# Molecolab-Pisa/diaglib

Measured on AMD Instinct MI355X. Metric: eigensolver GFLOP/s + iters-to-converge, n=2e6 m=8 Davidson, 1/2/4/8 GPU, higher is better.
Workload: dtype f64; 1 GPU; davidson n=2000000 roots=8 n_max=13 max_dav=20 tol=2e-13 operator=diag(i+1)+0.5*W*W^T(rank 4) guess=unit callbacks=device; workload_key=davidson n=2000000 roots=8 n_max=13 max_dav=20 guess=unit, iters=9, matvec_cols=105, restarts=0, converged=True, rows_per_gpu=2000000

## Files before the change

### diaglib_amd/csrc/hip_engine.hip

```cpp
#include <hip/hip_runtime.h>
#include <rccl/rccl.h>
#include <algorithm>
#include <cmath>
#include <cstdio>
#include <cstdlib>
#include <type_traits>
#include <utility>
#include <cstring>
#include <ctime>
#include <map>
#include <set>
#include <vector>
#include "dla_internal.h"
#include "hip_owned.h"
#include "hip_plans.h"

using namespace dla_plans;

typedef double v4d __attribute__((ext_vector_type(4)));
typedef double v2d __attribute__((ext_vector_type(2)));

template <int V> struct VecOf;
template <> struct VecOf<1> { typedef double type; };
template <> struct VecOf<2> { typedef v2d type; };
// ... 106 lines not shown
  };
  bool want[TLW][KT];
  bool any_want = false;
#pragma unroll
  for (int t = 0; t < TLW; ++t)
#pragma unroll
    for (int q = 0; q < KT; ++q) {
      want[t][q] = !a.lower || (xg * TLW + t >= ug * KT + q);
      any_want = any_want || want[t][q];
    }
  auto mfma_chunk = [&](const vec_t (&xd)[TLW][RSTEP], const vec_t (&ud)[KT][RSTEP]) {
#pragma unroll
    for (int s = 0; s < RSTEP; ++s)
#pragma unroll
      for (int e = 0; e < VEC; ++e)
#pragma unroll
        for (int t = 0; t < TLW; ++t)
#pragma unroll
          for (int q = 0; q < KT; ++q)
            if (want[t][q])
              acc[t][q] = __builtin_amdgcn_mfma_f64_16x16x4f64(vget<VEC>(xd[t][s], e), vget<VEC>(ud[q][s], e),
                                                               acc[t][q], 0, 0, 0);
  };
  if (!any_want) ch = (1LL << 62);
  if constexpr (PREFETCH) {
    if (ch < nfull) {
      load_chunk(ch, xv, uv);
      for (; ch + stride < nfull; ch += stride) {
        vec_t xn[TLW][RSTEP], un[KT][RSTEP];
        load_chunk(ch + stride, xn, un);
        mfma_chunk(xv, uv);
#pragma unroll
        for (int t = 0; t < TLW; ++t)
#pragma unroll
          for (int s = 0; s < RSTEP; ++s) xv[t][s] = xn[t][s];
#pragma unroll
        for (int q = 0; q < KT; ++q)
#pragma unroll
          for (int s = 0; s < RSTEP; ++s) uv[q][s] = un[q][s];
      }
      mfma_chunk(xv, uv);
      ch += stride;
    }
  } else {
    for (; ch < nfull; ch += stride) {
      load_chunk(ch, xv, uv);
      mfma_chunk(xv, uv);
    }
  }
  if (ch == nfull && nfull * CH < n) {
    const long long rbase = nfull * CH;
#pragma unroll
    for (int s = 0; s < RSTEP; ++s) {
      const bool ok = rbase + 4 * VEC * s + VEC * g < n;
#pragma unroll
      for (int q = 0; q < KT; ++q) {
        uv[q][s] = vzero<VEC>();
        if (ok) uv[q][s] = *(const vec_t*)(up[q] + rbase + 4 * VEC * s);
      }
#pragma unroll
      for (int t = 0; t < TLW; ++t) {
        xv[t][s] = vzero<VEC>();
        if (ok) xv[t][s] = *(const vec_t*)(xp[t] + rbase + 4 * VEC * s);
      }
    }
    mfma_chunk(xv, uv);
  }

  __shared__ double red[4][256];
  double* pout = a.partial + ((size_t)blockIdx.y * gridDim.x + blockIdx.x) * (size_t)(TLW * KT) * 256;
#pragma unroll
  for (int t = 0; t < TLW; ++t)
#pragma unroll
    for (int q = 0; q < KT; ++q) {
#pragma unroll
      for (int r = 0; r < 4; ++r) red[wave][r * 64 + lane] = acc[t][q][r];
      __syncthreads();
      double s = ((red[0][threadIdx.x] + red[1][threadIdx.x]) + red[2][threadIdx.x]) + red[3][threadIdx.x];
      pout[(size_t)(t * KT + q) * 256 + threadIdx.x] = s;
      __syncthreads();
    }
}

template <int TLW, int KT, int NT = 1, int R = 16, int SELF = 0, int QT = 0, int LOW = 0, int WP = 0>
__global__ __launch_bounds__(256) void gram_lds_kernel(GramArgs a)
{
  DLA_PREDICATED(a);
  static_assert(!WP || (QT == 0 && LOW == 0 && KT <= 3 && (KT == 1 || (!SELF && R == 16))), "pending factor: up to three U tiles");
  static_assert(WP != 2 || (KT == 1 && !SELF), "projection sweep: one U tile beside the X tiles");
  constexpr int UU = (WP && !SELF) ? KT * (KT + 1) / 2 : 0;
  constexpr int NSLOT = TLW * KT + UU;
  constexpr int RS = R + 2;
  constexpr int LPC = R / 2;
  constexpr int CPI = 64 / LPC;
  constexpr int NC = SELF ? 16 * TLW : 16 * (TLW + KT);
  constexpr int UOFF = SELF ? 0 : 16 * TLW;
  constexpr int NI = NC / CPI;
  extern __shared__ __attribute__((aligned(16))) double glds[];
  const int lane = threadIdx.x & 63, wave = threadIdx.x >> 6;
  double* my = glds + (size_t)wave * NC * RS;
  const int c = lane & 15, g = lane >> 4;
  const int li = lane % LPC, lc = lane / LPC;
  const int xg = blockIdx.y % a.passes_x, ug = blockIdx.y / a.passes_x;
  const long long n = a.n;

  v4d acc[TLW][KT];
  bool want[TLW][KT];
  bool any_want = false;
  unsigned tile_used = 0;
#pragma unroll
  for (int t = 0; t < TLW; ++t)
#pragma unroll
    for (int q = 0; q < KT; ++q) {
      acc[t][q] = (v4d){0.0, 0.0, 0.0, 0.0};
      const int xt = xg * TLW + t, ut = ug * KT + q;
      want[t][q] = (16 * xt < a.l) && (16 * ut < a.k) && (LOW ? (t >= q) : (!a.lower || xt >= ut));
      any_want = any_want || want[t][q];
      if (want[t][q]) tile_used |= (1u << t) | (1u << (SELF ? q : TLW + q));
    }
  const double* cp[NI];
  unsigned skip = 0;
#pragma unroll
  for (int j = 0; j < NI; ++j) {
    const int sc = CPI * j + lc;
    if (!(tile_used & (1u << ((CPI * j) / 16)))) skip |= 1u << j;
    if (sc < 16 * TLW) {
      int col = xg * TLW * 16 + sc;
      if (xg * TLW * 16 + CPI * j >= a.l) skip |= 1u << j;
      col = col < a.l ? col : a.l - 1;
      cp[j] = a.x + (size_t)col * (size_t)n + 2 * li;
    } else {
      int col = ug * KT * 16 + (sc - 16 * TLW);
      if (ug * KT * 16 + (CPI * j - 16 * TLW) >= a.k) skip |= 1u << j;
      col = col < a.k ? col : a.k - 1;
      cp[j] = a.u + (size_t)col * (size_t)n + 2 * li;
    }
  }
  if (a.noskip & 1) skip = 0;
  long long rmul[NI];
#pragma unroll
  for (int j = 0; j < NI; ++j) {
    rmul[j] = 1;
    if (skip & (1u << j)) { rmul[j] = 0; cp[j] = a.x; }
  }
  const int i4 = lane & 3;
  double accq[SELF ? KT : TLW][QT > 0 ? QT : 1];
#pragma unroll
  for (int t = 0; t < (SELF ? KT : TLW); ++t)
#pragma unroll
    for (int qq = 0; qq < (QT > 0 ? QT : 1); ++qq) accq[t][qq] = 0.0;
  v4d accuu[UU > 0 ? UU : 1];
#pragma unroll
  for (int e = 0; e < (UU > 0 ? UU : 1); ++e) accuu[e] = (v4d){0.0, 0.0, 0.0, 0.0};
  double wa[WP == 1 ? KT * (KT + 1) / 2 : 1][WP == 1 ? 4 : 1];
  double ca[WP == 2 ? 4 * (TLW + 1) : 1];
  if constexpr (WP == 2) {
#pragma unroll
    for (int s = 0; s < 4 * (TLW + 1); ++s) {
      const int sc = 4 * s + g;
      const int row = sc < 16 * TLW ? (sc < a.l ? sc : -1) : (sc - 16 * TLW < a.k ? a.l + sc - 16 * TLW : -1);
      ca[s] = row >= 0 ? a.cx[(size_t)row * 16 + c] : 0.0;
    }
  }
  if constexpr (WP == 1) {
    const int k4w = ((a.k + 3) / 4) * 4;
#pragma unroll
    for (int q = 0; q < KT; ++q)
#pragma unroll
      for (int p = 0; p <= q; ++p)
#pragma unroll
        for (int s = 0; s < 4; ++s) {
          const int pp = 16 * p + 4 * s + g;
          double v = (pp == 16 * q + c) ? 1.0 : 0.0;
          if (a.wp) v = (KT == 1) ? a.wp[pp * 16 + c] : (pp < k4w ? a.wp[((size_t)q * k4w + pp) * 16 + c] : 0.0);
          wa[q * (q + 1) / 2 + p][s] = v;
        }
  }
  typedef VecOf<2>::type vec_t;
  vec_t stg[NI];
  auto load_tile = [&](long long tile) {
    const long long r0 = tile * R;
    if constexpr (LOW) {
#pragma unroll
      for (int j = 0; j < NI; ++j) {
        const int sc = CPI * j + lc;
        const bool isx = sc < 16 * TLW;
        int col = isx ? sc : sc - 16 * TLW;
        col = col < a.l ? col : a.l - 1;
        const double* base = isx ? a.x : a.u;
        const bool pin = (isx ? CPI * j : CPI * j - 16 * TLW) >= a.l;
        stg[j] = pload<2, NT>(pin ? a.x : base + (size_t)col * (size_t)n + 2 * li + r0);
      }
    } else {
#pragma unroll
      for (int j = 0; j < NI; ++j) stg[j] = pload<2, NT>(cp[j] + r0 * rmul[j]);
    }
  };
  auto stage_tile = [&]() {
#pragma unroll
    for (int j = 0; j < NI; ++j) lds_store2(my + (size_t)(CPI * j + lc) * RS + 2 * li, stg[j]);
  };
  constexpr int KF = (QT > 0 && !SELF) ? KT - 1 : KT;
  constexpr int TF = (QT > 0 && SELF) ? TLW - 1 : TLW;
  auto apply_w = [&](long long r0w, bool rows_ok) {
    if constexpr (WP) {
      if (WP == 1 && a.wp == nullptr && a.uw == nullptr) return;
      double* ut = my + (size_t)UOFF * RS + c;
      if constexpr (WP == 2) {
        v4d d[R / 16];
#pragma unroll
        for (int h = 0; h < R / 16; ++h) d[h] = (v4d){0.0, 0.0, 0.0, 0.0};
#pragma unroll
        for (int s = 0; s < 4 * (TLW + 1); ++s)
#pragma unroll
          for (int h = 0; h < R / 16; ++h)
            d[h] = __builtin_amdgcn_mfma_f64_16x16x4f64(ca[s], lds_load1(my + (size_t)(4 * s + g) * RS + c + 16 * h), d[h], 0, 0, 0);
        __builtin_amdgcn_wave_barrier();
#pragma unroll
        for (int h = 0; h < R / 16; ++h)
#pragma unroll
          for (int r = 0; r < 4; ++r) lds_store1(ut + (size_t)(g + 4 * r) * RS + 16 * h, d[h][r]);
      } else if constexpr (KT == 1) {
        double uin[R / 16][4];
#pragma unroll
        for (int h = 0; h < R / 16; ++h)
#pragma unroll
          for (int s = 0; s < 4; ++s) uin[h][s] = lds_load1(ut + (size_t)(4 * s + g) * RS + 16 * h);
        v4d d[R / 16];
#pragma unroll
        for (int h = 0; h < R / 16; ++h) d[h] = (v4d){0.0, 0.0, 0.0, 0.0};
#pragma unroll
        for (int s = 0; s < 4; ++s)
#pragma unroll
          for (int h = 0; h < R / 16; ++h) d[h] = __builtin_amdgcn_mfma_f64_16x16x4f64(wa[0][s], uin[h][s], d[h], 0, 0, 0);
#pragma unroll
        for (int h = 0; h < R / 16; ++h)
#pragma unroll
          for (int r = 0; r < 4; ++r) lds_store1(ut + (size_t)(g + 4 * r) * RS + 16 * h, d[h][r]);
      } else {
        double uin[KT][4];
#pragma unroll
        for (int p = 0; p < KT; ++p)
#pragma unroll
          for (int s = 0; s < 4; ++s) uin[p][s] = lds_load1(ut + (size_t)(16 * p + 4 * s + g) * RS);
        v4d d[KT];
#pragma unroll
        for (int q = 0; q < KT; ++q) {
          d[q] = (v4d){0.0, 0.0, 0.0, 0.0};
#pragma unroll
          for (int p = 0; p <= q; ++p)
#pragma unroll
            for (int s = 0; s < 4; ++s) d[q] = __builtin_amdgcn_mfma_f64_16x16x4f64(wa[q * (q + 1) / 2 + p][s], uin[p][s], d[q], 0, 0, 0);
        }
        __builtin_amdgcn_wave_barrier();
#pragma unroll
        for (int q = 0; q < KT; ++q)
#pragma unroll
          for (int r = 0; r < 4; ++r) lds_store1(ut + (size_t)(16 * q + g + 4 * r) * RS, d[q][r]);
      }
      __builtin_amdgcn_wave_barrier();
      if (a.uw != nullptr && rows_ok) {
#pragma unroll
        for (int j = (16 * (SELF ? 0 : TLW)) / CPI; j < NI; ++j) {
          const int uc = CPI * j + lc - UOFF;
          if (uc < a.k) pstore<2, 0>(a.uw + (size_t)uc * (size_t)n + r0w + 2 * li, *(const lds_v2f64*)(my + (size_t)(CPI * j + lc) * RS + 2 * li));
        }
      }
    }
  };
  auto mfma_tile = [&]() {
#pragma unroll
    for (int s4 = 0; s4 < R / 4; ++s4) {
      double uf[KT];
#pragma unroll
      for (int q = 0; q < (SELF ? KT : KF); ++q) uf[q] = lds_load1(my + (size_t)(UOFF + 16 * q + c) * RS + 4 * s4 + g);
      if constexpr (UU > 0) {
#pragma unroll
        for (int qi = 0; qi < KT; ++qi)
#pragma unroll
          for (int qj = 0; qj <= qi; ++qj)
            accuu[qi * (qi + 1) / 2 + qj] = __builtin_amdgcn_mfma_f64_16x16x4f64(uf[qi], uf[qj], accuu[qi * (qi + 1) / 2 + qj], 0, 0, 0);
      }
      double uq[QT > 0 ? QT : 1];
      if constexpr (QT > 0 && !SELF) {
#pragma unroll
        for (int qq = 0; qq < QT; ++qq) uq[qq] = lds_load1(my + (size_t)(UOFF + 16 * KF + 4 * qq + i4) * RS + 4 * s4 + g);
      }
#pragma unroll
      for (int t = 0; t < TF; ++t) {
        const double xf = lds_load1(my + (size_t)(16 * t + c) * RS + 4 * s4 + g);
#pragma unroll
        for (int q = 0; q < KF; ++q)
          if (want[t][q]) acc[t][q] = __builtin_amdgcn_mfma_f64_16x16x4f64(xf, uf[q], acc[t][q], 0, 0, 0);
        if constexpr (QT > 0 && !SELF) {
#pragma unroll
          for (int qq = 0; qq < QT; ++qq)
            if (want[t][KT - 1]) accq[t][qq] = mfma_quarter(xf, uq[qq], accq[t][qq]);
        }
      }
      if constexpr (QT > 0 && SELF) {
#pragma unroll
        for (int qq = 0; qq < QT; ++qq) {
          const double xq = lds_load1(my + (size_t)(16 * TF + 4 * qq + i4) * RS + 4 * s4 + g);
#pragma unroll
          for (int q = 0; q < KT; ++q) accq[q][qq] = mfma_quarter(xq, uf[q], accq[q][qq]);
        }
      }
    }
  };
  const long long nfull = n / R;
  const long long stride = (long long)gridDim.x * 4;
  long long tile = (long long)blockIdx.x * 4 + wave;
  if (!any_want) tile = (1LL << 62);
  if (tile < nfull) {
    load_tile(tile);
    for (;;) {
      stage_tile();
      __builtin_amdgcn_wave_barrier();
      const long long next = tile + stride;
      if (next < nfull) load_tile(next);
      apply_w(tile * R, true);
      mfma_tile();
      __builtin_amdgcn_wave_barrier();
      tile = next;
      if (next >= nfull) break;
    }
  }
  if (tile == nfull && nfull * R < n) {
    const long long r0 = nfull * R;
    const bool ok = r0 + 2 * li < n;
#pragma unroll
    for (int j = 0; j < NI; ++j) {
      stg[j] = vzero<2>();
      if (ok) stg[j] = *(const vec_t*)(cp[j] + r0 * rmul[j]);
    }
    stage_tile();
    __builtin_amdgcn_wave_barrier();
    apply_w(r0, ok);
    mfma_tile();
    __builtin_amdgcn_wave_barrier();
  }

  __syncthreads();
  double* red = glds;
  double* pout = a.partial + ((size_t)blockIdx.y * gridDim.x + blockIdx.x) * (size_t)NSLOT * 256;
  if constexpr (UU > 0) {
#pragma unroll
    for (int e = 0; e < UU; ++e) {
#pragma unroll
      for (int r = 0; r < 4; ++r) red[wave * 256 + r * 64 + lane] = accuu[e][r];
      __syncthreads();
      pout[(size_t)(TLW * KT + e) * 256 + threadIdx.x] = ((red[threadIdx.x] + red[256 + threadIdx.x]) + red[512 + threadIdx.x]) + red[768 + threadIdx.x];
      __syncthreads();
    }
  }
#pragma unroll
  for (int t = 0; t < TLW; ++t)
#pragma unroll
    for (int q = 0; q < KT; ++q) {
      if (LOW && t < q) {
        pout[(size_t)(t * KT + q) * 256 + threadIdx.x] = 0.0;
        continue;
      }
      if (QT > 0 && !SELF && q == KT - 1) {
#pragma unroll
        for (int r = 0; r < 4; ++r) red[wave * 256 + r * 64 + lane] = 0.0;
#pragma unroll
        for (int qq = 0; qq < QT; ++qq) red[wave * 256 + ((lane >> 2) & 3) * 64 + 16 * g + 4 * qq + i4] = accq[t][qq];
      } else if (QT > 0 && SELF && t == TLW - 1) {
#pragma unroll
        for (int r = 0; r < 4; ++r) red[wave * 256 + r * 64 + lane] = r < QT ? accq[q][r < QT ? r : 0] : 0.0;
      } else {
#pragma unroll
        for (int r = 0; r < 4; ++r) red[wave * 256 + r * 64 + lane] = acc[t][q][r];
      }
      __syncthreads();
      double sum = ((red[threadIdx.x] + red[256 + threadIdx.x]) + red[512 + threadIdx.x]) + red[768 + threadIdx.x];
      pout[(size_t)(t * KT + q) * 256 + threadIdx.x] = sum;
      __syncthreads();
    }
}

struct GemmArgs {
  const double* x;
  const double* cpk;
  double* z;
  double* gpart;
  long long n;
  int l, l4, k;
  const int* phase;
  int want;
  int xpf;
};

struct GemmArgsInl {
  const double* x;
  double* z;
  double* gpart;
  long long n;
  int l, l4, k;
  const int* phase;
  int want;
  int xpf;
  double cin[256];
};
__device__ __forceinline__ const double* packed_c(const GemmArgs& a) { return a.cpk; }
__device__ __forceinline__ const double* packed_c(const GemmArgsInl& a) { return a.cin; }

template <int KT, int VEC, int MODE, typename ARGS, bool GRAM = false, int NT = (MODE == 2 ? 0 : 1), int PIPE = (KT >= 2 ? 2 : 0), int ZPAD = 9,
          int QT = 0, int RTP = 2>
__global__ __launch_bounds__(256) void gemm_kernel(ARGS a)
{
  DLA_PREDICATED(a);
  constexpr int RT = RTP;
  constexpr int RG = 16 * VEC;
  constexpr int WT = RT * RG;
  extern __shared__ __attribute__((aligned(16))) double cs[];
  typedef typename VecOf<VEC>::type vec_t;
  const long long n = a.n;
// ... 3170 lines not shown
  int reduce_and_sum(int cls, double* c, double* c_host, int nblk, int l, int k, int tlw, int kt, int px, int n_out, int extra, int ldc,
                     StepOut& out)
  {
    Rode rode;
    {
      Scope s2(this, cls, 0.0, 0.0, "gram_reduce_kernel");
      const int groups = reduce_groups(nblk);
      { const int stl = ensure_lvl2(sizeof(double) * (size_t)n_out * groups * 256); if (stl) return stl; }
      if (n_out > 4096) { err = "gram: too many output tiles"; return DLA_ERR_ARG; }
      GramReduceArgs ra{d_partial, d_lvl2, d_ticket, c, c_host, nblk, l, k, tlw, kt, px,
                        lc.phase, lc.want, 0, n_out, d_ticket + 4096, OrthoTailArgs{}, P2PArgs{}, extra, ldc};
      rode = launch_reduce(ra, dim3(n_out, groups));
    }
    HIPCHK(hipGetLastError());
    out.tail_fused = rode.tail;
    if (lc.in_chunk) return DLA_OK;
    return allreduce_dev(c, (ldc ? ldc : l) * k, 0, h_small, out, rode.exchange);
  }
  void launch_tail_kernel(const OrthoTailArgs& ta)
  {
    if (ta.fold) DLA_LAUNCH(ortho_tail16_kernel, dim3(1), dim3(256), 0, st, ta);
    else DLA_LAUNCH(ortho_tail_kernel, dim3(1), dim3(64), 0, st, ta);
  }

  int launch_op(int op, int n, int m, int k, const double* x, const double* bx, double* u, bool publish, int fold)
  {
    OrthoTailArgs tail{d_ost, h_ost.dev(), d_small, d_wpk, d_wfull, d_cpk2, op, m, k, m > 0 ? 1 : 0, ortho_maxit, publish ? 1 : 0,
                       fold, knobs.lead_full() ? 0 : 1, d_xug, d_wst, d_dbg, lc.xw ? 1 : 0};
    if ((fold == 1 && op == OP_GRAMX) || op == OP_XW || op == OP_COMBOX) tail.gsrc = d_xug;
    tail.x3 = lc.x3 ? 1 : 0;
    tail.gp = knobs.first_factor_source();
    tail.dmat = (policy.basis_exact && fold && m > 0 && dmat_nontrivial && dmat_cols == m && m <= DMAT_LD) ? d_dmat : nullptr;
    tail.dmat_ld = DMAT_LD;
    tail.drop_final = (policy.drop_final && m > 0) ? 1 : 0;
    tail.t_host = (tail.drop_final && policy.publish_pending && m + k <= PEND_ROWS) ? h_tpend.dev() : nullptr;
    tail.t_seq = t_seq;
    tail.drop_tol = policy.drop_tol;
    tail.drop_stol = policy.drop_stol;
    StepOut out;
    int stc = DLA_OK;
    {
      LaunchCtx step = lc;
      step.fuse_tail = p2p.on ? !knobs.exchange_own_launch() : (nranks <= 1 && !comm);
      step.tail = tail;
      step.phase = &d_ost->phase;
      step.want = (op == OP_GRAMX) ? (int)OP_GRAM_UU : (lc.x3 && op == OP_COMBO) ? (int)OP_COMBOX : op;
      CtxScope scope(this, step);
      int blocks = 0;
      switch (op) {
        case OP_GRAM_UU: stc = gram_dev_once(n, k, u, k, u, DLA_OP_GRAM, false, out); break;
        case OP_XU:      stc = gram_dev_once(n, m, bx, k, u, DLA_OP_GRAM, false, out); break;
        case OP_GRAMX:
          stc = fold == 1 ? gram_wp_once(n, m, bx, k, u, nullptr, nullptr, out) : gram_dev_once(n, m + k, x, k, u, DLA_OP_GRAM, false, out);
          break;
        case OP_XW:      stc = gram_wp_once(n, m, bx, k, u, d_wpk, u, out); break;
        case OP_GRAMW:   stc = gram_wp_once(n, 0, nullptr, k, u, d_wpk, nullptr, out); break;
        case OP_TRMMG:
        case OP_TRMMC:
          stc = gemm_chunk(n, 0, k, u, k, nullptr, 0, u, 2, DLA_OP_TRMM, &blocks, d_wpk);
          if (!stc) stc = fused_reduce(k, blocks, out);
          break;
        case OP_COMBO:
          stc = gemm_chunk(n, 0, m + k, x, k, nullptr, 0, u, 0, DLA_OP_GEMM, &blocks, d_cpk2);
          if (!stc) stc = fused_reduce(k, blocks, out);
          break;
        case OP_FINAL:   stc = gemm_chunk(n, 0, k, u, k, nullptr, 0, u, 2, DLA_OP_TRMM, nullptr, d_wpk); break;
        case OP_COMBOX:  stc = gram_wp_once(n, m, bx, k, u, nullptr, u, out, d_cpk2); break;
        case OP_CLOSE:   stc = gemm_chunk(n, 0, m + k, x, k, nullptr, 0, u, 0, DLA_OP_GEMM, nullptr, d_cpk2); break;
        default: err = "ortho_chain: bad op"; stc = DLA_ERR_ARG;
      }
    }
    if (stc || out.tail_fused) return stc;
    if (comm && !p2p.on && d_red_small) {
      if (out.summed_at) tail.gsrc = out.summed_at;
      tail.xug = d_red_xug;
    }
    Scope s(this, DLA_OP_GRAM, 0.0, 0.0, fold ? "ortho_tail16_kernel" : "ortho_tail_kernel");
    launch_tail_kernel(tail);
    HIPCHK(hipGetLastError());
    return DLA_OK;
  }

  template <int TLW, int KT, int R>
  int launch_gram_wp(const GramArgs& a, dim3 grid, bool self)
  {
    if (a.cx != nullptr) {
      if constexpr (KT == 1) {
        auto kfn = gram_lds_kernel<TLW, 1, 1, R, 0, 0, 0, 2>;
        const size_t lds = gram_lds_bytes(TLW, 1, R, false, false);
        if (!raise_lds((const void*)kfn, lds)) return DLA_ERR_RUNTIME;
        DLA_LAUNCH(kfn, grid, dim3(256), lds, st, a);
        return DLA_OK;
      }
      err = "gram_wp: the projection sweep takes one-tile blocks"; return DLA_ERR_ARG;
    }
    if (self) {
      if constexpr (TLW == 1 && KT == 1) {
        auto kfn = gram_lds_kernel<1, 1, 1, 32, 1, 0, 0, 1>;
        const size_t lds = gram_lds_bytes(1, 1, 32, true, false);
        DLA_LAUNCH(kfn, grid, dim3(256), lds, st, a);
      }
      return DLA_OK;
    }
    auto kfn = gram_lds_kernel<TLW, KT, 1, R, 0, 0, 0, 1>;
    const size_t lds = gram_lds_bytes(TLW, KT, R, false, false);
    if (!raise_lds((const void*)kfn, lds)) return DLA_ERR_RUNTIME;
    DLA_LAUNCH(kfn, grid, dim3(256), lds, st, a);
    return DLA_OK;
  }
  int gram_wp_once(int n, int m, const double* x, int k, const double* u, const double* wp, double* uw, StepOut& out, const double* cx = nullptr)
  {
    out = StepOut{};
    const bool self = (m == 0);
    if (cx != nullptr && (self || uw == nullptr || wp != nullptr || k > 16)) { err = "gram_wp: bad projection sweep"; return DLA_ERR_ARG; }
    if (k > 48 || (self && k > 16)) { err = "gram_wp: block too wide"; return DLA_ERR_ARG; }
    const WpPlan p = wp_plan(env(), n, m, k, cx != nullptr);
    const int tlw = p.tlw, kt = p.kt, passes = p.passes, blocks = p.blocks, extra = p.extra, slots = p.slots;
    int stc = ensure_partial(sizeof(double) * (size_t)passes * blocks * slots * 256);
    if (stc) return stc;
    stc = ensure_small(sizeof(double) * (size_t)k * k);
    if (stc) return stc;
    if (!self && (m + k) * k > XUG_DOUBLES) { err = "gram_wp: basis too wide for the chain's buffer"; return DLA_ERR_ARG; }
    if (uw != nullptr && passes != 1) { err = "gram_wp: the storing sweep takes one pass"; return DLA_ERR_ARG; }
    GramArgs a{self ? u : x, u, d_partial, (long long)n, self ? k : m, k, passes, 0, lc.phase, lc.want, 0, wp, uw, cx};
    dim3 grid(blocks, passes);
    {
      Scope s(this, cx ? DLA_OP_GEMM : DLA_OP_GRAM, 8.0 * (double)n * (double)(m + k + (uw ? k : 0)),
              2.0 * (double)n * (m + k) * k + ((wp || cx) ? 1.0 * (double)n * k * k : 0.0) + (cx ? 2.0 * (double)n * m * k : 0.0), p.name());
      int r_ = DLA_ERR_RUNTIME;
      if (!first_instance<std::size(WP_TILES)>([&](auto i) {
            constexpr WpTile s = WP_TILES[decltype(i)::value];
            if (tlw != s.tlw || kt != s.kt || p.R != s.R) return false;
            r_ = launch_gram_wp<s.tlw, s.kt, s.R>(a, grid, self);
            return true;
          }))
        err = "gram_wp: no kernel instance";
      if (r_) return r_;
    }
    const int n_out = self ? 1 : passes * tlw * kt + extra;
    return reduce_and_sum(DLA_OP_GRAM, self ? d_small : d_xug, nullptr, blocks, self ? k : m, k, tlw, kt, passes, n_out, extra, self ? k : m + k, out);
  }

  struct ChainRun {
    bool active = false;
    int n = 0, m = 0, k = 0, fold = 0;
    bool vsx = false;
    const double *x = nullptr, *bx = nullptr;
    double* u = nullptr;
    ChainShape shape;
    bool xw = false;
    bool x3 = false;
    bool lean = false;
    std::vector<int> plan, launched;
    std::vector<SpecRec> recs;
  } run;

  DeviceBuffer<double> d_dmat;
  std::vector<std::vector<double>> h_dcols;
  int dmat_cols = 0;
  bool dmat_nontrivial = false;
  int basis_state(int m) const override { return m <= 0 ? 0 : dmat_cols != m ? -1 : dmat_nontrivial ? 1 : 0; }
  int basis_capacity() const override { return DMAT_LD; }
  bool basis_exact_ok() const override { return !hook && !local_only && !knobs.no_exact_basis() && lds_limit > (size_t)128 * 1024; }
  int basis_dd(int m, int k, double* xu, int ld) override
  {
    if (!policy.basis_exact || m <= 0) return DLA_OK;
    if (dmat_cols != m) { err = "ortho_vs_x: the copy of the caller's pending blocks does not describe this basis (dla_basis_sync after every block)"; return DLA_ERR_ARG; }
    if (!dmat_nontrivial) return DLA_OK;
    std::vector<double> y(m);
    for (int j = 0; j < k; ++j) {
      double* s = xu + (size_t)j * ld;
      for (int r = 0; r < m; ++r) {
        const double* dr = h_dcols[r].data();
        double acc = 0.0;
        for (int i = 0; i <= r; ++i) acc += dr[i] * s[i];
        y[r] = acc;
      }
      for (int i = 0; i < m; ++i) s[i] = 0.0;
      for (int q = 0; q < m; ++q) {
        const double* dq = h_dcols[q].data();
        const double yq = y[q];
        for (int i = 0; i <= q; ++i) s[i] += dq[i] * yq;
      }
    }
    return DLA_OK;
  }
  int basis_sync(int m, int k, const double* dmat, int ld) override
  {
    if (k <= 0) { dmat_cols = 0; dmat_nontrivial = false; h_dcols.clear(); return DLA_OK; }
    if (m != dmat_cols) { err = "basis_sync: the blocks of D arrive in order (" + std::to_string(dmat_cols) + " columns known, block starts at " + std::to_string(m) + ")"; return DLA_ERR_ARG; }
    h_dcols.resize((size_t)m + k);
    for (int j = 0; j < k; ++j) {
      std::vector<double>& col = h_dcols[(size_t)m + j];
      col.resize((size_t)m + j + 1);
      for (int i = 0; i <= m + j; ++i) {
        const double v = dmat[(size_t)i + (size_t)(m + j) * ld];
        col[i] = v;
        if (v != (i == m + j ? 1.0 : 0.0)) dmat_nontrivial = true;
      }
    }
    dmat_cols = m + k;
    if (m + k > DMAT_LD) return DLA_OK;
    bind();
    { const int stz = reserve_zeroed(d_dmat, (size_t)DMAT_LD * DMAT_LD); if (stz) return stz; }
    double* h = nullptr;
    int slot = 0;
    const size_t bytes = sizeof(double) * (size_t)k * DMAT_LD;
    const int stc = stage_slot(bytes, &h, &slot);
    if (stc) return stc;
    std::memset(h, 0, bytes);
    for (int j = 0; j < k; ++j) std::memcpy(h + (size_t)j * DMAT_LD, h_dcols[(size_t)m + j].data(), sizeof(double) * (size_t)(m + j + 1));
    return stage_commit(slot, bytes, d_dmat + (size_t)m * DMAT_LD);
  }

  int pending_block(int m, int k, double* p, int ldp, int* applied) override
  {
// ... 230 lines not shown
          std::printf("    op %llu (err est %.2e, max|G-I| %.2e, max|X^T U| %.2e (col sq %.2e), chol %llu cycles = %.2f GHz): kernel entry->tail %.2f us | G load %.2f | chol+inv %.2f | norms %.2f | products+stores %.2f | decide %.2f | publish %.2f | assemble %.2f\n",
                      q[9], 2.2e-16 * rc * rc, gdev, sdev, csq, q[11], us(1, 2) > 0 ? (double)q[11] / (us(1, 2) * 1e3) : 0.0, us(8, 0), us(0, 1), us(1, 2), us(2, 3), us(3, 4), us(4, 5), us(5, 6), us(6, 7));
        }
        (void)hipMemset(d_dbg, 0, sizeof(unsigned long long) * 48 * 16);
      }
    }
    {
      const int nlog = std::min(sres.nops, 48);
      ChainDone cd;
      cd.launched.swap(launched); cd.recs.swap(recs);
      std::copy(sres.log, sres.log + nlog, cd.log);
      cd.nlog = nlog; cd.n = n; cd.k = k;
      unaccounted.push_back(std::move(cd));
      if (sres.status == OST_DONE && sres.nops <= 48) { hist.assign(sres.log, sres.log + nlog); last_k = hist; }
    }
    if (sres.status == OST_DONE && policy.publishes() && vsx && h_tpend[PEND_HDR] == (double)t_seq) t_pending_k = k;
    rep->handled = 1;
    rep->status = sres.status;
    rep->growth = sres.growth;
    rep->outer_its = sres.it_outer;
    rep->macro_its = sres.macro_total;
    rep->shifts = sres.shifts;
    return DLA_OK;
  }

  DeviceBuffer<int> d_bgo; MappedHostBuffer<int> h_bstat; DeviceBuffer<double> d_wpk_b;
  int b_seq = 0;
  int b_ortho_ahead(int n, int k, double* u, double* bu, bool behind_chain, int* handled) override
  {
    *handled = 0;
    if (k <= 0 || k > 48 || hook || local_only || knobs.no_b_ortho_ahead()) return DLA_OK;
    bind();
    { const int stz = reserve_zeroed(d_bgo, 1); if (stz) return stz; }
    HIPCHK(h_bstat.reserve(1));
    HIPCHK(d_wpk_b.reserve(3 * 48 * 16));
    int stc = ensure_chain_buffers();
    if (stc) return stc;
    StepOut gram_out;
    stc = gram_dev(n, k, u, k, bu, gram_out);
    if (stc) return stc;
    b_seq = b_seq >= 1000000 ? 1 : b_seq + 1;
    *h_bstat = 0;
    {
      Scope s(this, DLA_OP_GRAM, 0.0, 0.0, "bortho_tail_kernel");
      BOrthoTailArgs ta{d_ost, d_small, d_wpk_b, k, behind_chain ? 1 : 0, b_seq, d_bgo, h_bstat.dev()};
      DLA_LAUNCH(bortho_tail_kernel, dim3(1), dim3(64), 0, st, ta);
      HIPCHK(hipGetLastError());
    }
    {
      LaunchCtx behind = lc;
      behind.phase = d_bgo; behind.want = b_seq;
      CtxScope scope(this, behind);
      stc = gemm_chunk(n, 0, k, u, k, nullptr, 0, u, 2, DLA_OP_TRMM, nullptr, d_wpk_b);
      if (!stc) stc = gemm_chunk(n, 0, k, bu, k, nullptr, 0, bu, 2, DLA_OP_TRMM, nullptr, d_wpk_b);
    }
    if (stc) return stc;
    *handled = 1;
    return DLA_OK;
  }
  int b_ortho_ahead_status() override
  {
    const int v = *(volatile int*)h_bstat;
    return v == b_seq ? 1 : (v == -b_seq ? -1 : 0);
  }

  template <int TLW, int KT, int R>
  int launch_gram_lds(const GramArgs& a, dim3 grid, const GramPlan& p)
  {
#define GLK(SELF_, Q)                                                                                          \
    do {                                                                                                      \
      auto kfn = gram_lds_kernel<TLW, KT, 1, R, SELF_, Q>;                                                    \
      const size_t lds = gram_lds_bytes(TLW, KT, R, SELF_, false);                                            \
      if (!raise_lds((const void*)kfn, lds)) return DLA_ERR_RUNTIME;                                          \
      DLA_LAUNCH(kfn, grid, dim3(256), lds, st, a);                                                   \
      return DLA_OK;                                                                                          \
    } while (0)
    if constexpr (TLW == KT) {
      if (p.self) {
        if constexpr (KT >= 2) { if (p.qt == 1) GLK(1, 1); if (p.qt == 2) GLK(1, 2); }
        GLK(1, 0);
      }
    }
    if constexpr (KT >= 2) { if (p.qt == 1) GLK(0, 1); if (p.qt == 2) GLK(0, 2); }
    GLK(0, 0);
#undef GLK
  }
  template <int T>
  int launch_gram_low(const GramArgs& a, dim3 grid, const GramPlan& p)
  {
    auto kfn = gram_lds_kernel<T, T, 1, 16, 0, 0, 1>;
    const size_t lds = gram_lds_bytes(T, T, 16, false, true);
    if (!raise_lds((const void*)kfn, lds)) return DLA_ERR_RUNTIME;
    DLA_LAUNCH(kfn, grid, dim3(256), lds, st, a);
    return DLA_OK;
  }
  template <int TLW, int KT>
  int launch_gram(const GramArgs& a, dim3 grid, const GramPlan& p)
  {
    if constexpr (KT <= 3) {
      if (p.lds) {
        if constexpr (gram_can32(TLW, KT)) { if (p.rows == 32) return launch_gram_lds<TLW, KT, 32>(a, grid, p); }
        return launch_gram_lds<TLW, KT, 16>(a, grid, p);
      }
    }
    if constexpr (!gram_direct_instance(TLW, KT)) {
      err = "gram: width without a direct-load instance";
      return DLA_ERR_RUNTIME;
    } else {
      constexpr int RS = gram_rs(TLW, KT);
      if (p.vec2) DLA_LAUNCH((gram_kernel<TLW, KT, 2, RS>), grid, dim3(256), 0, st, a);
      else      DLA_LAUNCH((gram_kernel<TLW, KT, 1, RS>), grid, dim3(256), 0, st, a);
      return DLA_OK;
    }
  }

  int gram_dev(int n, int l, const double* x, int k, const double* u, StepOut& out, int cls = DLA_OP_GRAM, bool lower = false)
  {
    return with_lds_retry([&]() { return gram_dev_once(n, l, x, k, u, cls, lower, out); });
  }
  int gram_dev_once(int n, int l, const double* x, int k, const double* u, int cls, bool lower, StepOut& out)
  {
    out = StepOut{};
    const GramPlan p = gram_plan(env(), n, l, k, x == u, peers_even && ((uintptr_t)x | (uintptr_t)u) % 16 == 0, lower);
    const int tlw = p.tlw, kt = p.kt, passes = p.passes, blocks_per_pass = p.blocks_per_pass;
    out.lower_only = p.self;
    const int slots = tlw * kt;
    int stc = ensure_partial(sizeof(double) * (size_t)passes * blocks_per_pass * slots * 256);
    if (stc) return stc;
    stc = ensure_small(sizeof(double) * (size_t)l * k);
    if (stc) return stc;
    GramArgs a{x, u, d_partial, (long long)n, l, k, p.px, p.lower ? 1 : 0, lc.phase, lc.want, knobs.gram_load_pads() ? 1 : 0};
    dim3 grid(blocks_per_pass, passes);
    {
      const bool same = (x == u) && (l == k);
      Scope s(this, cls, 8.0 * (double)n * (same ? (double)k : (double)(l + k)), 2.0 * (double)n * l * k, p.name());
      int r_ = DLA_ERR_RUNTIME;
      const bool hit = p.low_single ? first_instance<std::size(GRAM_LOW_TILES)>([&](auto i) {
                                        constexpr int T = GRAM_LOW_TILES[decltype(i)::value];
                                        if (tlw != T) return false;
                                        r_ = launch_gram_low<T>(a, grid, p);
                                        return true;
                                      })
                                    : first_instance<std::size(GRAM_TILES)>([&](auto i) {
                                        constexpr GramTile s = GRAM_TILES[decltype(i)::value];
                                        if (tlw != s.tlw || kt != s.kt) return false;
                                        r_ = launch_gram<s.tlw, s.kt>(a, grid, p);
                                        return true;
                                      });
      if (!hit) err = "gram: no kernel instance";
      if (r_) return r_;
    }
    return reduce_and_sum(cls, d_small + lc.small_off, lc.phase ? nullptr : h_small.dev() + lc.small_off, blocks_per_pass, l, k, tlw, kt, p.px,
                          passes * slots, 0, 0, out);
  }

  Event ev_chunk;
  bool gram_chunks_ok(int n, int l, int k) override
  {
    (void)n;
    return !hook && !comm && !p2p.on && (local_only || nranks <= 1) && l > 0 && k > 0 && lc.phase == nullptr;
  }
  int gram_chunk(int n, int l, const double* x, int k_total, int c0, int kc, const double* u_chunk) override
  {
    if (c0 == 0) { int stc = ensure_small(sizeof(double) * (size_t)l * k_total); if (stc) return stc; }
    HIPCHK(ev_chunk.ensure(hipEventDisableTiming));
    HIPCHK(hipEventRecord(ev_chunk, st_up));
// ... 1173 lines not shown
```

### diaglib_amd/csrc/hip_plans.h

```cpp
#pragma once
#include <algorithm>
#include <cstddef>
#include <cstdio>
#include <iterator>
#include <string>
#include <tuple>
#include <vector>
#include "dla_internal.h"

namespace dla_plans {

struct Knobs {
  int tune[8] = {0, 0, 0, 0, 0, 0, 0, 0};
  void set(int i, int v) { if (i >= 0 && i < 8) tune[i] = v; }
  int get(int i) const { return (i >= 0 && i < 8) ? tune[i] : 0; }
  int ritz_pipe_depth() const { return tune[0] == 1 ? 0 : tune[0] == 4 ? 4 : -1; }
  bool ritz_p_separate() const { return tune[0] == 5; }
  bool no_ritz2() const { return tune[0] == 6; }
  int ritz_grid_factor() const { return tune[1] > 0 ? tune[1] : 1; }
  int gemm_pipe_depth() const { return tune[2] == 1 ? 0 : tune[2] == 4 ? 4 : -1; }
  int gemm_blocks_per_cu() const { return tune[3] > 0 ? tune[3] : 0; }
  int gram_blocks_override() const { return tune[4] > 0 ? tune[4] : 0; }
  bool wp_one_block_per_cu() const { return tune[4] == -1; }
  bool direct_gram() const { return tune[5] == 2; }
  bool fenced_reduce() const { return tune[5] == 3; }
  bool poll_stream() const { return tune[6] == 2; }
  bool host_loop() const { return tune[6] == 3; }
  bool exchange_own_launch() const { return tune[6] == 4; }
  bool no_mfma_kxk() const { return tune[6] == 5; }
  bool no_pending_factor() const { return tune[6] == 6; }
  bool no_wide_gramx() const { return tune[6] == 7 || tune[6] == 8; }
  bool lead_full() const { return tune[6] == 7; }
  bool no_wide_xw() const { return tune[6] == 9; }
  bool wide_xw_three_tiles() const { return tune[6] == 10; }
  bool no_b_ortho_ahead() const { return tune[6] == 11; }
  bool five_sweep() const { return tune[6] == 12; }
  bool three_pass_always() const { return tune[6] == 13; }
  bool mode5_as_mode4() const { return tune[6] == 14; }
  bool no_exact_basis() const { return host_loop() || no_mfma_kxk() || mode5_as_mode4(); }
  int first_factor_source() const { return tune[6] == 15 ? 0 : tune[6] == 16 ? 2 : 1; }
  bool keep_closing_launches() const { return tune[6] == 17; }
  bool no_quarter_tiles() const { return tune[7] == 1; }
  bool gram_load_pads() const { return tune[7] == 2; }
  bool narrow_gram_passes() const { return tune[7] == 3; }
  bool no_next_tile_prefetch() const { return tune[7] == 4; }
  bool fused3_two_row_groups() const { return tune[7] == 5; }
  bool no_low_single() const { return tune[7] == 8; }
  bool own_copy_kernel() const { return tune[7] == 9; }
  int reduce_group_size() const { return tune[7] == 22 ? 16 : tune[7] == 23 ? 64 : 32; }
};

constexpr int DMAT_LD = 320, XUG_DOUBLES = 640 * 16, P2P_MAX_DOUBLES = 16384, PEND_ROWS = 640;

struct PlanEnv { int ncu; size_t lds_limit; const Knobs& knobs; };

template <typename... A>
inline std::string plan_name(const char* fmt, A... a)
{
  char kn[96];
  std::snprintf(kn, sizeof kn, fmt, a...);
  return kn;
}

inline int quarter_tiles(const PlanEnv& env, int k, bool vec2)
{
  const int kt = (k + 15) / 16, rem = k - 16 * (kt - 1);
  return (vec2 && kt >= 2 && kt <= 3 && rem <= 8 && !env.knobs.no_quarter_tiles()) ? (rem + 3) / 4 : 0;
}
inline int blocks_per_cu(size_t lds) { return lds > 80 * 1024 ? 1 : lds > 40 * 1024 ? 2 : 4; }

struct GramTile { int tlw, kt; };
constexpr GramTile GRAM_TILES[] = {
  {1, 1}, {2, 1}, {3, 1}, {4, 1}, {5, 1}, {6, 1}, {7, 1}, {8, 1}, {10, 1}, {12, 1},
  {1, 2}, {2, 2}, {3, 2}, {4, 2}, {5, 2}, {6, 2}, {7, 2}, {8, 2},
  {1, 3}, {2, 3}, {3, 3}, {4, 3}, {5, 3}, {6, 3}, {7, 3},
  {1, 4}, {2, 4}, {3, 4}};
constexpr bool gram_direct_instance(int tlw, int kt)
{
  return !(tlw == 5 || tlw == 7 || tlw == 10 || (tlw == 12 && kt > 1) || (tlw == 3 && kt >= 2 && kt <= 3) || (tlw >= 5 && kt == 3) ||
           (tlw >= 7 && kt == 2));
}
constexpr int GRAM_LOW_TILES[] = {4, 5, 6, 7};
struct WpTile { int tlw, kt, R; };
constexpr WpTile WP_TILES[] = {
  {1, 1, 32}, {2, 1, 32}, {3, 1, 16}, {4, 1, 16}, {5, 1, 16}, {6, 1, 16}, {7, 1, 16}, {8, 1, 16}, {10, 1, 16}, {12, 1, 16},
  {1, 2, 16}, {2, 2, 16}, {3, 2, 16}, {4, 2, 16}, {5, 2, 16}, {6, 2, 16}, {7, 2, 16}, {8, 2, 16},
  {1, 3, 16}, {2, 3, 16}, {3, 3, 16}, {4, 3, 16}, {5, 3, 16}};
struct RitzInstance { int kt, vec, pipe, qt; bool xp; };
constexpr RitzInstance RITZ_INSTANCES[] = {
  {2, 2, 2, 1, true}, {3, 2, 3, 1, true}, {2, 2, 2, 2, true}, {3, 2, 3, 2, true},
  {1, 2, 0, 0, true}, {2, 2, 2, 0, true}, {3, 2, 3, 0, true}, {4, 2, 3, 0, true}, {5, 2, 3, 0, true},
  {2, 2, 0, 0, false}, {3, 2, 0, 0, false}, {2, 2, 4, 0, false}, {3, 2, 4, 0, false},
  {2, 2, 2, 1, false}, {3, 2, 3, 1, false}, {2, 2, 2, 2, false}, {3, 2, 3, 2, false},
  {1, 2, 0, 0, false}, {2, 2, 2, 0, false}, {3, 2, 3, 0, false},
  {1, 1, 0, 0, false}, {2, 1, 2, 0, false}, {3, 1, 3, 0, false}};
template <typename Tile, size_t N, typename Ok>
constexpr const Tile* listed_pass(const Tile (&list)[N], int kt, int want, Ok ok)
{
  const Tile* best = nullptr;
  for (const Tile& t : list)
    if (t.kt == kt && t.tlw >= want && ok(t) && (!best || t.tlw < best->tlw)) best = &t;
  return best;
}

constexpr bool gram_can32(int tlw, int kt) { return sizeof(double) * 4 * 16 * (tlw + kt) * 34 <= 150 * 1024 && tlw + kt <= 7; }
constexpr int gram_rs(int tlw, int kt) { return (tlw * kt >= 6) ? 2 : 4; }
inline int lds_rows(const PlanEnv& env, int tlw, int kt)
{
  const int r = ((tlw <= 2 || kt == 3) && tlw + kt <= 7) ? 32 : 16;
  return (r == 32 && sizeof(double) * 4 * 16 * (size_t)(tlw + kt) * 34 > env.lds_limit) ? 16 : r;
}
inline bool use_lds_gram(const PlanEnv& env, bool vec2, int l, int kt) { return vec2 && kt <= 3 && l > 8 && !env.knobs.direct_gram(); }

constexpr size_t gram_lds_bytes(int tlw, int kt, int rows, bool self, bool low)
{
  return sizeof(double) * 4 * 16 * (size_t)(low ? 2 * tlw : self ? tlw : tlw + kt) * (size_t)(rows + 2);
}
struct GramPlan {
  int tlw, kt;
  int px, passes;
  int rows;
  bool lds;
  bool self;
  int qt;
  bool low_single;
  bool lower;
  int blocks_per_pass;
  bool vec2;
  std::string name() const
  {
    if (lds) return plan_name("gram_lds_kernel<%d, %d, 1, %d, %d, %d, %d, 0>", tlw, kt, rows, self ? 1 : 0, qt, low_single ? 1 : 0);
    return plan_name("gram_kernel<%d, %d, %d, %d, 0, -1>", tlw, kt, vec2 ? 2 : 1, gram_rs(tlw, kt));
  }
  size_t lds_bytes() const { return lds ? gram_lds_bytes(tlw, kt, rows, self, low_single) : 0; }
};
inline GramPlan gram_plan(const PlanEnv& env, int n, int l, int k, bool same, bool aligned, bool lower)
{
  const Knobs& knobs = env.knobs;
  const int tx = (l + 15) / 16, tu = (k + 15) / 16;
  const bool vec2 = n % 2 == 0 && aligned;
  int kt = std::min(tu, (vec2 && l > 8 && !knobs.direct_gram()) ? 3 : 4);
  const int passes_u = (tu + kt - 1) / kt;
  kt = (tu + passes_u - 1) / passes_u;
  const bool ldsk = use_lds_gram(env, vec2, l, kt);
  static const int maxtl[5] = {0, 8, 6, 4, 3};
  static const int maxtl_lds[4] = {0, 12, 8, 7};
  int mt = ldsk ? maxtl_lds[kt] : maxtl[kt];
  if (knobs.narrow_gram_passes()) mt = (ldsk && kt == 1) ? 12 : maxtl[kt];
  if (ldsk) mt = std::max(1, std::min(mt, (int)(env.lds_limit / (sizeof(double) * 4 * 16 * 18)) - kt));
  const int passes_x = (tx + mt - 1) / mt;
  int tlw = (tx + passes_x - 1) / passes_x;
  if (const GramTile* t = listed_pass(GRAM_TILES, kt, tlw, [&](const GramTile& g) { return ldsk || gram_direct_instance(g.tlw, g.kt); })) tlw = t->tlw;
  int px = (tx + tlw - 1) / tlw;
  int passes = px * passes_u;
  const bool self = ldsk && same && l == k && passes == 1 && tlw == kt;
  if (self) lower = true;
  int qt = (ldsk && passes_u == 1 && kt >= 2) ? quarter_tiles(env, k, vec2) : 0;
  const bool low_single = lower && ldsk && !self && l == k && tx >= 4 && tx <= 7 && passes > 1 && !knobs.no_low_single() &&
                          sizeof(double) * 4 * 16 * (size_t)(2 * tx) * 18 <= env.lds_limit;
  if (low_single) { kt = tlw = tx; px = 1; passes = 1; qt = 0; }
  const int ch = vec2 ? 32 : 16;
  long long nchunks = ((long long)n + ch - 1) / ch;
  long long want = (nchunks + 4 * 4 - 1) / (4 * 4);
  int blocks_per_pass = (int)std::max(1LL, std::min((long long)env.ncu, want));
  if (tlw * kt == 1 && ((same && l == k) || l <= 8)) blocks_per_pass = (int)std::max(1LL, std::min(2LL * env.ncu, want));
  if (knobs.gram_blocks_override()) blocks_per_pass = (int)std::max(1LL, std::min((long long)knobs.gram_blocks_override(), want));
  const int rows = (ldsk && !low_single && gram_can32(tlw, kt) && lds_rows(env, tlw, kt) == 32) ? 32 : 16;
  return GramPlan{tlw, kt, px, passes, rows, ldsk, self, qt, low_single, lower, blocks_per_pass, vec2};
}

inline int wp_max_tlw(int kt) { return kt <= 1 ? 12 : kt == 2 ? 8 : 5; }
struct WpPlan {
  int tlw, kt, R, passes, blocks, extra, slots;
  bool self;
  bool project;
  std::string name() const { return plan_name("gram_lds_kernel<%d, %d, 1, %d, %d, 0, 0, %d>", tlw, kt, R, self ? 1 : 0, project ? 2 : 1); }  size_t lds_bytes() const { return gram_lds_bytes(tlw, kt, R, self, false); }
};
inline WpPlan wp_plan(const PlanEnv& env, int n, int m, int k, bool project)
{
  const Knobs& knobs = env.knobs;
  WpPlan p{};
  p.self = (m == 0);
  p.project = project;
  p.kt = (k + 15) / 16;
  const int tx = p.self ? 1 : (m + 15) / 16;
  p.passes = p.self ? 1 : (tx + wp_max_tlw(p.kt) - 1) / wp_max_tlw(p.kt);
  p.tlw = (tx + p.passes - 1) / p.passes;
  p.R = 16;
  if (const WpTile* t = listed_pass(WP_TILES, p.kt, p.tlw, [](const WpTile&) { return true; })) { p.tlw = t->tlw; p.R = t->R; }
  const long long nchunks = ((long long)n + 31) / 32;
  const long long want = (nchunks + 15) / 16;
  p.blocks = (int)std::max(1LL, std::min((long long)env.ncu * ((p.self || (p.kt == 1 && p.tlw <= 5 && !knobs.wp_one_block_per_cu())) ? 2 : 1), want));
  if (knobs.gram_blocks_override()) p.blocks = (int)std::max(1LL, std::min((long long)knobs.gram_blocks_override(), want));
  p.extra = p.self ? 0 : p.kt * (p.kt + 1) / 2;
  p.slots = p.self ? 1 : p.tlw * p.kt + p.extra;
  return p;
}

struct GemmPlan {
  int kt, l4;
  bool inl;
  int qt;
  size_t lds;
  int per_cu, rtp, pipe, blocks;
  bool vec2, fuse;
  int mode;
  std::string name() const
  {
    return plan_name("gemm_kernel<%d, %d, %d, %s, %s, %d, %d, 9, %d, %d>", kt, vec2 ? 2 : 1, mode, inl ? "GemmArgsInl" : "GemmArgs",
                     fuse ? "true" : "false", mode == 2 ? 0 : 1, pipe, qt, rtp);
  }
};
inline GemmPlan gemm_plan(const PlanEnv& env, int n, int l, int k, int mode, bool fuse, bool packed_on_device, bool vec2)
{
  const Knobs& knobs = env.knobs;
  const int kt = (k + 15) / 16;
  const int l4 = ((l + 3) / 4) * 4;
  const bool inl = (!packed_on_device && kt == 1 && l4 <= 16);
  const int ab_depth = fuse ? -1 : knobs.gemm_pipe_depth();
  int qt = ab_depth >= 0 ? 0 : quarter_tiles(env, k, vec2);
  if (!fuse && mode == 1 && kt == 2) qt = 0;
  const size_t lds_c = sizeof(double) * (size_t)l4 * (qt > 0 ? 16 * (kt - 1) + 8 : 16 * kt);
  const size_t lds = fuse ? std::max(lds_c + sizeof(double) * 4 * 16 * (16 * kt + 9), (size_t)8192) : lds_c;
  int per_cu = blocks_per_cu(lds);
  if (knobs.gemm_blocks_per_cu()) per_cu = (int)std::max((size_t)1, std::min((size_t)knobs.gemm_blocks_per_cu(), (size_t)(156 * 1024) / std::max(lds, (size_t)4096)));
  const int rtp = (fuse && kt == 3 && vec2 && per_cu >= 2 && !knobs.fused3_two_row_groups()) ? 1 : 2;
  const int pipe = (ab_depth >= 0 && vec2 && kt >= 2 && (mode == 0 || mode == 1)) ? ab_depth : (fuse && kt >= 3) ? 3 : kt >= 2 ? 2 : 0;
  const int wt = (vec2 ? 32 : 16) * rtp;
  const long long ntiles = ((long long)n + wt - 1) / wt;
  const int blocks = (int)std::max(1LL, std::min((long long)env.ncu * per_cu, (ntiles + 3) / 4));
  return GemmPlan{kt, l4, inl, qt, lds, per_cu, rtp, pipe, blocks, vec2, fuse, mode};
}

inline size_t fused_lds(int l, int k)
{
  const int kt = (k + 15) / 16, l4 = ((l + 3) / 4) * 4;
  return std::max(sizeof(double) * ((size_t)kt * l4 * 16 + (size_t)4 * 16 * (16 * kt + 9)), (size_t)8192);
}

inline size_t ritz_lds_cap(int kt) { return (size_t)(kt >= 4 ? 100 : 150) * 1024; }
inline size_t ritz_static_lds(int kt) { return (size_t)1024 + (kt >= 4 ? sizeof(double) * 4 * 48 * 16 * 2 : 0); }
inline size_t ritz_dyn_limit(const PlanEnv& env, int kt)
{
  const size_t st_ = ritz_static_lds(kt);
  return std::min(ritz_lds_cap(kt), env.lds_limit > st_ ? env.lds_limit - st_ : (size_t)0);
}
struct RitzGrid {
  size_t lds;
  int per_cu, blocks;
  int ncol, nslots;
  size_t small_doubles() const { return (size_t)ncol * (1 + nslots); }
};
inline RitzGrid ritz_grid(const PlanEnv& env, int n, bool vec2, int kt, size_t lds_c, int grid_factor, int nranks_slots)
{
  const int rg = vec2 ? 32 : 16;
  const long long ntiles = ((long long)n + rg - 1) / rg;
  const size_t lds = std::max(lds_c, sizeof(double) * 4 * 16 * kt * 2);
  const int per_cu = blocks_per_cu(lds);
  const int blocks = (int)std::max(1LL, std::min((long long)env.ncu * per_cu * grid_factor, (ntiles + 7) / 8));
  return RitzGrid{lds, per_cu, blocks, 16 * kt, nranks_slots};
}
struct RitzPlan : RitzGrid {
  int kt;
  int l4, qt;
  bool xp;
  int pipe;
  size_t lds_c;
  bool fits;
  bool vec2;
  std::string name() const { return plan_name("ritz_kernel<%d, %d, 3, %d, %d, %s, 0>", kt, vec2 ? 2 : 1, pipe, qt, xp ? "true" : "false"); }
};
inline RitzPlan ritz_plan(const PlanEnv& env, int n, int l, int m, int k2, bool vec2, int nranks_slots)
{
  const Knobs& knobs = env.knobs;
  RitzPlan p{};
  p.vec2 = vec2;
// ... 149 lines not shown
```

Baseline: 13900 GFLOP/s.

## Add two-stage register prefetch to LDS Gram and pending-factor sweep kernels

Adds a DEPTH=2 variant of gram_lds_kernel that keeps two tiles of global loads in flight, using alternating register buffers and a software-pipelined loop unrolled by two. It is enabled by default for single-U-tile Gram plans and for wide pending-factor/projection sweeps, with a knob to fall back to one stage. The goal is to hide HBM latency behind the MFMA and LDS work on the memory-bound tall-skinny reductions. The cost is more registers per thread, which may lower occupancy, plus extra kernel instantiations.

New measurement: 13740 GFLOP/s. -1.2%, worse.

```diff
diff --git a/diaglib_amd/csrc/hip_engine.hip b/diaglib_amd/csrc/hip_engine.hip
--- a/diaglib_amd/csrc/hip_engine.hip
+++ b/diaglib_amd/csrc/hip_engine.hip
@@ -212,10 +212,11 @@
     }
 }
 
-template <int TLW, int KT, int NT = 1, int R = 16, int SELF = 0, int QT = 0, int LOW = 0, int WP = 0>
+template <int TLW, int KT, int NT = 1, int R = 16, int SELF = 0, int QT = 0, int LOW = 0, int WP = 0, int DEPTH = 1>
 __global__ __launch_bounds__(256) void gram_lds_kernel(GramArgs a)
 {
   DLA_PREDICATED(a);
+  static_assert(DEPTH == 1 || (DEPTH == 2 && KT == 1 && !SELF && !LOW && QT == 0), "second load stage: one U tile, plain or pending-factor sweeps");
   static_assert(!WP || (QT == 0 && LOW == 0 && KT <= 3 && (KT == 1 || (!SELF && R == 16))), "pending factor: up to three U tiles");
   static_assert(WP != 2 || (KT == 1 && !SELF), "projection sweep: one U tile beside the X tiles");
   constexpr int UU = (WP && !SELF) ? KT * (KT + 1) / 2 : 0;
@@ -308,7 +309,7 @@
   }
   typedef VecOf<2>::type vec_t;
   vec_t stg[NI];
-  auto load_tile = [&](long long tile) {
+  auto load_tile = [&](long long tile, vec_t (&stg)[NI]) __attribute__((always_inline)) {
     const long long r0 = tile * R;
     if constexpr (LOW) {
 #pragma unroll
@@ -326,13 +327,13 @@
       for (int j = 0; j < NI; ++j) stg[j] = pload<2, NT>(cp[j] + r0 * rmul[j]);
     }
   };
-  auto stage_tile = [&]() {
+  auto stage_tile = [&](const vec_t (&stg)[NI]) __attribute__((always_inline)) {
 #pragma unroll
     for (int j = 0; j < NI; ++j) lds_store2(my + (size_t)(CPI * j + lc) * RS + 2 * li, stg[j]);
   };
   constexpr int KF = (QT > 0 && !SELF) ? KT - 1 : KT;
   constexpr int TF = (QT > 0 && SELF) ? TLW - 1 : TLW;
-  auto apply_w = [&](long long r0w, bool rows_ok) {
+  auto apply_w = [&](long long r0w, bool rows_ok) __attribute__((always_inline)) {
     if constexpr (WP) {
       if (WP == 1 && a.wp == nullptr && a.uw == nullptr) return;
       double* ut = my + (size_t)UOFF * RS + c;
@@ -398,7 +399,7 @@
       }
     }
   };
-  auto mfma_tile = [&]() {
+  auto mfma_tile = [&]() __attribute__((always_inline)) {
 #pragma unroll
     for (int s4 = 0; s4 < R / 4; ++s4) {
       double uf[KT];
@@ -442,13 +443,57 @@
   const long long stride = (long long)gridDim.x * 4;
   long long tile = (long long)blockIdx.x * 4 + wave;
   if (!any_want) tile = (1LL << 62);
-  if (tile < nfull) {
-    load_tile(tile);
+  if constexpr (DEPTH == 2) {
+    vec_t stg2[NI];
+    auto one_tile = [&](long long t) __attribute__((always_inline)) {
+      apply_w(t * R, true);
+      mfma_tile();
+      __builtin_amdgcn_wave_barrier();
+    };
+    if (tile < nfull) {
+      load_tile(tile, stg);
+      if (tile + stride < nfull) {
+        load_tile(tile + stride, stg2);
+        while (tile + 3 * stride < nfull) {
+          stage_tile(stg);
+          __builtin_amdgcn_wave_barrier();
+          load_tile(tile + 2 * stride, stg);
+          one_tile(tile);
+          stage_tile(stg2);
+          __builtin_amdgcn_wave_barrier();
+          load_tile(tile + 3 * stride, stg2);
+          one_tile(tile + stride);
+          tile += 2 * stride;
+        }
+        const bool third = tile + 2 * stride < nfull;
+        stage_tile(stg);
+        __builtin_amdgcn_wave_barrier();
+        if (third) load_tile(tile + 2 * stride, stg);
+        one_tile(tile);
+        stage_tile(stg2);
+        __builtin_amdgcn_wave_barrier();
+        one_tile(tile + stride);
+        tile += 2 * stride;
+        if (third) {
+          stage_tile(stg);
+          __builtin_amdgcn_wave_barrier();
+          one_tile(tile);
+          tile += stride;
+        }
+      } else {
+        stage_tile(stg);
+        __builtin_amdgcn_wave_barrier();
+        one_tile(tile);
+        tile += stride;
+      }
+    }
+  } else if (tile < nfull) {
+    load_tile(tile, stg);
     for (;;) {
-      stage_tile();
+      stage_tile(stg);
       __builtin_amdgcn_wave_barrier();
       const long long next = tile + stride;
-      if (next < nfull) load_tile(next);
+      if (next < nfull) load_tile(next, stg);
       apply_w(tile * R, true);
       mfma_tile();
       __builtin_amdgcn_wave_barrier();
@@ -464,7 +509,7 @@
       stg[j] = vzero<2>();
       if (ok) stg[j] = *(const vec_t*)(cp[j] + r0 * rmul[j]);
     }
-    stage_tile();
+    stage_tile(stg);
     __builtin_amdgcn_wave_barrier();
     apply_w(r0, ok);
     mfma_tile();
@@ -3801,12 +3846,21 @@
   }
 
   template <int TLW, int KT, int R>
-  int launch_gram_wp(const GramArgs& a, dim3 grid, bool self)
-  {
+  int launch_gram_wp(const GramArgs& a, dim3 grid, bool self, int depth)
+  {
+    if (depth != 1 && !wp_depth2_instance(TLW, KT, a.cx != nullptr)) { err = "gram_wp: no two-stage instance of this width"; return DLA_ERR_RUNTIME; }
     if (a.cx != nullptr) {
       if constexpr (KT == 1) {
+        const size_t lds = gram_lds_bytes(TLW, 1, R, false, false);
+        if constexpr (wp_depth2_instance(TLW, KT, true)) {
+          if (depth == 2) {
+            auto kfn2 = gram_lds_kernel<TLW, 1, 1, R, 0, 0, 0, 2, 2>;
+            if (!raise_lds((const void*)kfn2, lds)) return DLA_ERR_RUNTIME;
+            DLA_LAUNCH(kfn2, grid, dim3(256), lds, st, a);
+            return DLA_OK;
+          }
+        }
         auto kfn = gram_lds_kernel<TLW, 1, 1, R, 0, 0, 0, 2>;
-        const size_t lds = gram_lds_bytes(TLW, 1, R, false, false);
         if (!raise_lds((const void*)kfn, lds)) return DLA_ERR_RUNTIME;
         DLA_LAUNCH(kfn, grid, dim3(256), lds, st, a);
         return DLA_OK;
@@ -3821,8 +3875,16 @@
       }
       return DLA_OK;
     }
+    const size_t lds = gram_lds_bytes(TLW, KT, R, false, false);
+    if constexpr (wp_depth2_instance(TLW, KT, false)) {
+      if (depth == 2) {
+        auto kfn2 = gram_lds_kernel<TLW, KT, 1, R, 0, 0, 0, 1, 2>;
+        if (!raise_lds((const void*)kfn2, lds)) return DLA_ERR_RUNTIME;
+        DLA_LAUNCH(kfn2, grid, dim3(256), lds, st, a);
+        return DLA_OK;
+      }
+    }
     auto kfn = gram_lds_kernel<TLW, KT, 1, R, 0, 0, 0, 1>;
-    const size_t lds = gram_lds_bytes(TLW, KT, R, false, false);
     if (!raise_lds((const void*)kfn, lds)) return DLA_ERR_RUNTIME;
     DLA_LAUNCH(kfn, grid, dim3(256), lds, st, a);
     return DLA_OK;
@@ -3850,7 +3912,7 @@
       if (!first_instance<std::size(WP_TILES)>([&](auto i) {
             constexpr WpTile s = WP_TILES[decltype(i)::value];
             if (tlw != s.tlw || kt != s.kt || p.R != s.R) return false;
-            r_ = launch_gram_wp<s.tlw, s.kt, s.R>(a, grid, self);
+            r_ = launch_gram_wp<s.tlw, s.kt, s.R>(a, grid, self, self ? 1 : p.depth);
             return true;
           }))
         err = "gram_wp: no kernel instance";
@@ -4247,6 +4309,15 @@
       }
     }
     if constexpr (KT >= 2) { if (p.qt == 1) GLK(0, 1); if (p.qt == 2) GLK(0, 2); }
+    if constexpr (gram_depth2_instance(TLW, KT, R)) {
+      if (p.depth == 2 && !p.self) {
+        auto kfn2 = gram_lds_kernel<TLW, KT, 1, R, 0, 0, 0, 0, 2>;
+        const size_t lds2 = gram_lds_bytes(TLW, KT, R, false, false);
+        if (!raise_lds((const void*)kfn2, lds2)) return DLA_ERR_RUNTIME;
+        DLA_LAUNCH(kfn2, grid, dim3(256), lds2, st, a);
+        return DLA_OK;
+      }
+    }
     GLK(0, 0);
 #undef GLK
   }
diff --git a/diaglib_amd/csrc/hip_plans.h b/diaglib_amd/csrc/hip_plans.h
--- a/diaglib_amd/csrc/hip_plans.h
+++ b/diaglib_amd/csrc/hip_plans.h
@@ -24,6 +24,7 @@
   bool wp_one_block_per_cu() const { return tune[4] == -1; }
   bool direct_gram() const { return tune[5] == 2; }
   bool fenced_reduce() const { return tune[5] == 3; }
+  bool single_stage_gram() const { return tune[5] == 4; }
   bool poll_stream() const { return tune[6] == 2; }
   bool host_loop() const { return tune[6] == 3; }
   bool exchange_own_launch() const { return tune[6] == 4; }
@@ -86,6 +87,8 @@
   {1, 1, 32}, {2, 1, 32}, {3, 1, 16}, {4, 1, 16}, {5, 1, 16}, {6, 1, 16}, {7, 1, 16}, {8, 1, 16}, {10, 1, 16}, {12, 1, 16},
   {1, 2, 16}, {2, 2, 16}, {3, 2, 16}, {4, 2, 16}, {5, 2, 16}, {6, 2, 16}, {7, 2, 16}, {8, 2, 16},
   {1, 3, 16}, {2, 3, 16}, {3, 3, 16}, {4, 3, 16}, {5, 3, 16}};
+constexpr bool gram_depth2_instance(int tlw, int kt, int rows) { return kt == 1 && (rows == 16 || tlw <= 2); }
+constexpr bool wp_depth2_instance(int tlw, int kt, bool project) { return kt == 1 && tlw >= 6 && tlw <= (project ? 8 : 10); }
 struct RitzInstance { int kt, vec, pipe, qt; bool xp; };
 constexpr RitzInstance RITZ_INSTANCES[] = {
   {2, 2, 2, 1, true}, {3, 2, 3, 1, true}, {2, 2, 2, 2, true}, {3, 2, 3, 2, true},
@@ -127,6 +130,7 @@
   bool lower;
   int blocks_per_pass;
   bool vec2;
+  int depth;
   std::string name() const
   {
     if (lds) return plan_name("gram_lds_kernel<%d, %d, 1, %d, %d, %d, %d, 0>", tlw, kt, rows, self ? 1 : 0, qt, low_single ? 1 : 0);
@@ -166,7 +170,8 @@
   if (tlw * kt == 1 && ((same && l == k) || l <= 8)) blocks_per_pass = (int)std::max(1LL, std::min(2LL * env.ncu, want));
   if (knobs.gram_blocks_override()) blocks_per_pass = (int)std::max(1LL, std::min((long long)knobs.gram_blocks_override(), want));
   const int rows = (ldsk && !low_single && gram_can32(tlw, kt) && lds_rows(env, tlw, kt) == 32) ? 32 : 16;
-  return GramPlan{tlw, kt, px, passes, rows, ldsk, self, qt, low_single, lower, blocks_per_pass, vec2};
+  const int depth = (ldsk && !self && !low_single && passes == 1 && gram_depth2_instance(tlw, kt, rows) && !knobs.single_stage_gram()) ? 2 : 1;
+  return GramPlan{tlw, kt, px, passes, rows, ldsk, self, qt, low_single, lower, blocks_per_pass, vec2, depth};
 }
 
 inline int wp_max_tlw(int kt) { return kt <= 1 ? 12 : kt == 2 ? 8 : 5; }
@@ -174,6 +179,7 @@
   int tlw, kt, R, passes, blocks, extra, slots;
   bool self;
   bool project;
+  int depth;
   std::string name() const { return plan_name("gram_lds_kernel<%d, %d, 1, %d, %d, 0, 0, %d>", tlw, kt, R, self ? 1 : 0, project ? 2 : 1); }  size_t lds_bytes() const { return gram_lds_bytes(tlw, kt, R, self, false); }
 };
 inline WpPlan wp_plan(const PlanEnv& env, int n, int m, int k, bool project)
@@ -192,6 +198,7 @@
   const long long want = (nchunks + 15) / 16;
   p.blocks = (int)std::max(1LL, std::min((long long)env.ncu * ((p.self || (p.kt == 1 && p.tlw <= 5 && !knobs.wp_one_block_per_cu())) ? 2 : 1), want));
   if (knobs.gram_blocks_override()) p.blocks = (int)std::max(1LL, std::min((long long)knobs.gram_blocks_override(), want));
+  p.depth = (!p.self && wp_depth2_instance(p.tlw, p.kt, project) && !knobs.single_stage_gram()) ? 2 : 1;
   p.extra = p.self ? 0 : p.kt * (p.kt + 1) / 2;
   p.slots = p.self ? 1 : p.tlw * p.kt + p.extra;
   return p;
```
